# qdrant/qdrant

Measured on AMD Instinct MI355X. Metric: QPS @ recall@10, brute-force, d=768 10M vecs, f32 cosine top-10, higher is better.
Workload: dtype f32 (int8 prefilter + exact f32 re-score)

## Files before the change

### qdrant_amd/csrc/api_core.hip

```cpp
#include "api_internal.hpp"

namespace qmx {

static thread_local std::string g_last_error;
const std::string &last_error_text() { return g_last_error; }

void set_error(const char *fmt, ...) {
    char buf[1024];
    va_list ap;
    va_start(ap, fmt);
    vsnprintf(buf, sizeof(buf), fmt, ap);
    va_end(ap);
    g_last_error = buf;
}

int32_t hip_status(hipError_t e, const char *what, const char *file, int line) {
    set_error("HIP error %d (%s) at %s:%d: %s", (int)e, hipGetErrorString(e), file, line, what);
    (void)hipGetLastError();
    switch (e) {
        case hipErrorOutOfMemory: return QMX_ERR_OUT_OF_MEMORY;
        case hipErrorNoDevice:
        case hipErrorInvalidDevice:
        case hipErrorNoBinaryForGpu:
        case hipErrorInsufficientDriver: return QMX_ERR_NO_DEVICE;
        case hipErrorNotReady: return QMX_ERR_NOT_READY;
        case hipErrorInvalidValue: return QMX_ERR_BAD_ARG;
        default: return QMX_ERR_OTHER;
    }
}

static const char *const g_option_names[OPT_COUNT] = {"no_mfma_scan", "no_mfma16", "no_prescan", "prescan_shift", "hnsw_log_cap", "no_split_scan", "split_min_queries", "no_split256", "no_pq_pair", "no_pq_prefilter", "pq_prefilter_min_queries", "hnsw_pq_per_cu", "tq_rotate_block", "no_topk_small", "verify_max_per_query", "hnsw_pq_direct_walk", "hnsw_pq_table_build", "hnsw_no_pq_prefilter", "hnsw_no_lds_visited", "pq_lut_no_lds", "hnsw_per_cu", "hnsw_reference_heap_order", "tq_wide_min_queries", "tq_wide_high_digit", "sq_wide_min_queries", "i8_resident", "i8_dense_epilogue", "i8_sample_stride", "prescan_beside_scan", "group_matrix_bytes", "debug"};
struct OptionTable {
    std::atomic<int64_t> v[OPT_COUNT];
    int64_t initial[OPT_COUNT];
    OptionTable() {
        for (int i = 0; i < OPT_COUNT; ++i) {
            char env[64] = "QMX_";
            size_t k = 4;
            for (const char *c = g_option_names[i]; *c && k + 1 < sizeof(env); ++c) env[k++] = (char)toupper((unsigned char)*c);
            env[k] = 0;
            const char *e = getenv(env);
            int64_t val = 0;
            if (e) { val = (*e >= '0' && *e <= '9') ? atoll(e) : 1; }
            if (i == OPT_PRESCAN_SHIFT && !e) val = 10;
            if (i == OPT_SPLIT_MIN_QUERIES && !e) val = 1;
            if (i == OPT_PQ_PREFILTER_MIN_QUERIES && !e) val = 4;
            if (i == OPT_TQ_WIDE_MIN_QUERIES && !e) val = 33;
            if (i == OPT_SQ_WIDE_MIN_QUERIES && !e) val = 33;
            if (i == OPT_I8_RESIDENT && !e) val = 1;
            if (i == OPT_I8_DENSE_EPILOGUE && !e) val = 1;
            if (i == OPT_I8_SAMPLE_STRIDE && !e) val = 16;
            if (i == OPT_PRESCAN_BESIDE_SCAN && !e) val = 1;
            initial[i] = val;
            v[i].store(val, std::memory_order_relaxed);
        }
    }
};
static OptionTable g_options;
int64_t option(Option o) { return g_options.v[o].load(std::memory_order_relaxed); }

static thread_local const void *g_last_kernel = nullptr;
const void *last_noted_kernel() { return g_last_kernel; }
void note_kernel(const void *host_function) { g_last_kernel = host_function; }

void clear_stale_error() {
    hipError_t e = hipGetLastError();
    if (e != hipSuccess) {
        const bool debug = option(OPT_DEBUG) != 0;
        if (debug) fprintf(stderr, "[qmx] dropped stale HIP error %d (%s) before a kernel launch\n", (int)e, hipGetErrorString(e));
    }
}

bool is_device_ptr(const void *p) {
    if (!p) return false;
// ... 91 lines not shown
```

### qdrant_amd/csrc/api_internal.hpp

```cpp
#pragma once
#include <stdarg.h>
#include <stdio.h>
#include <stdlib.h>
#include <string.h>

#include <ctype.h>
#include <cxxabi.h>

#include <algorithm>
#include <atomic>
#include <mutex>
#include <string>
#include <thread>
#include <new>
#include <vector>

#include "kernels.hpp"
#include "dev_mem.hpp"
#include "tq_rotate.hpp"

namespace qmx {
const std::string &last_error_text();
const void *last_noted_kernel();
bool is_device_ptr(const void *p);
// ... 123 lines not shown
    uint32_t timing_launches = 0;
    DevBuf partial, out, counts, ids, scores, misc, enc, bounds, gthr;
    DevBuf mv_qfirst, mv_offsets, mv_deleted;
    DevBuf cq_multi;
    DevBuf cq_sims, cq_scores, cq_desc, cq_coefs;
    uint32_t n_cq_coefs = 0;
    DevBuf cand, cand_cnt, cand_ids;
    DevBuf mmr_ids, mmr_rel;
    DevBuf grp_state, grp_pages, grp_scores, grp_queries, grp_partial, grp_out;
    DevBuf mmr_spill;
    DevBuf sp_bq, sp_f32, sp_cand, sp_cnt, sp_ver, sp_vscores, sp_sample, sp_wl, xcnt, tq_rot;
    DevBuf sh_lists, sh_out;
    std::vector<uint32_t> sh_bases_host;
    hipEvent_t sh_done = nullptr;
    hipEvent_t sh_merged = nullptr;
    DevBuf pq_table;
    DevBuf sp_probe, sp_pscores;
    DevBuf sp_plan, sp_fq;
    qmx_counters last_counters{};
    bool last_split = false, last_pq = false;
    uint32_t last_fqt = 64;
    uint64_t last_row_bytes = 0, last_n_cand = 0;
    uint64_t sp_sample_n = 0, sp_sample_of = 0;
    DevBuf filter;
    uint64_t n_filter_bits = 0;
    bool has_filter = false;
    DevBuf filter_of, filter_of_packed;
    uint32_t n_filters = 0;
    uint64_t filter_stride = 0;
    bool has_filters = false;
    DevBuf hnsw_lutx;
    DevBuf hnsw_pq8;
    DevBuf hnsw_next;
    DevBuf hnsw_refc;
    DevBuf hnsw_vis, hnsw_log, hnsw_scored;
    uint32_t hnsw_slots = 0;
    uint64_t hnsw_vis_words = 0;
    int *d_err = nullptr;
    uint32_t partial_grid_cap = 0;
    bool timing = false;
    const void *last_kernel = nullptr;
    SparseQuery *sparse = nullptr;

    qmx_query() = default;
    qmx_query(const qmx_query &) = delete;
    qmx_query &operator=(const qmx_query &) = delete;
// ... 284 lines not shown
```

### qdrant_amd/csrc/api_search.hip

```cpp
#include "api_internal.hpp"

extern "C" {

struct SearchCall {
    qmx_query *q;
    uint32_t top;
    const uint32_t *d_ids;
    uint64_t n_cand;
    qmx_scored_point *d_out;
    uint32_t *d_counts;
    const volatile uint8_t *is_stopped;
    qmx_counters *counters;
    bool timed;
    uint32_t launches;
};

static ScanArgs tile_args(const qmx_query *q, uint32_t top, uint64_t n_cand, uint32_t tile0, uint32_t nq_tile) {
    ScanArgs a;
    fill_args(q, tile0, nq_tile, a);
    a.n_cand = n_cand;
    a.top = top;
    return a;
}
static ScanArgs tile_args(const SearchCall &c, uint32_t tile0, uint32_t nq_tile) { return tile_args(c.q, c.top, c.n_cand, tile0, nq_tile); }
// ... 69 lines not shown
    hipError_t e = hipStreamSynchronize(q->stream);
    fprintf(stderr, "[qmx] split stage %-28s %s\n", what, e == hipSuccess ? "ok" : hipGetErrorString(e));
    fflush(stderr);
    QMX_HIP(e);
    return QMX_OK;
}

static int32_t verify_pool(qmx_query *q, unsigned char *plan, VerifyPool *vp) {
    const uint32_t cap = (uint32_t)std::min<uint64_t>(std::max<uint64_t>((uint64_t)q->nq * SPLIT_VCAP, 262144), 1u << 26);
    QMX_TRY(q->sp_ver.reserve(((size_t)cap * 2 + (size_t)q->nq * 2) * 4));
    QMX_TRY(q->sp_vscores.reserve((size_t)cap * 4));
    uint32_t *b = (uint32_t *)q->sp_ver.p;
    const int64_t mx = option(OPT_VERIFY_MAX_PER_QUERY);
    *vp = VerifyPool{b, b + cap, b + (size_t)2 * cap, b + (size_t)2 * cap + q->nq, (uint32_t *)(plan + SplitPlanLayout::pool_used), cap,
                     mx > 0 ? (uint32_t)std::min<int64_t>(mx, cap) : cap};
    return QMX_OK;
}

__global__ void sample_ids_kernel(uint32_t *ids, uint32_t n, uint64_t step) {
    const uint32_t i = blockIdx.x * blockDim.x + threadIdx.x;
    if (i < n) ids[i] = (uint32_t)((uint64_t)i * step);
}

static int32_t prefilter_begin(qmx_query *q, const SplitPlanLayout &pl, uint64_t n_cand, int shift, VerifyPool *vp, uint64_t *S_out) {
    QMX_TRY(q->sp_plan.reserve(pl.bytes));
    QMX_TRY(verify_pool(q, (unsigned char *)q->sp_plan.p, vp));
    const int sshift = (int)std::min<int64_t>(std::max<int64_t>(option(OPT_PRESCAN_SHIFT) + shift, 1), 20);
    const uint64_t S = std::min<uint64_t>(n_cand, std::max<uint64_t>(n_cand >> sshift, 8192));
    if (q->sp_sample_n != S || q->sp_sample_of != n_cand) {
        QMX_TRY(q->sp_sample.reserve((size_t)S * 4));
        ::qmx::clear_stale_error();
        hipLaunchKernelGGL(sample_ids_kernel, dim3((uint32_t)((S + 255) / 256)), dim3(256), 0, q->stream, (uint32_t *)q->sp_sample.p, (uint32_t)S, n_cand / S);
        QMX_HIP(hipGetLastError());
        q->sp_sample_n = S;
        q->sp_sample_of = n_cand;
    }
    QMX_HIP(hipMemsetAsync(q->sp_plan.p, 0, pl.zero_bytes, q->stream));
    *S_out = S;
    return QMX_OK;
}

static int32_t bound_enqueue(const SearchCall &c, uint32_t tile0, uint32_t nq_tile, const uint32_t *d_ids, uint64_t n, uint32_t ktop, const DeletedView &del,
                             uint32_t *launches, bool sample) {
    qmx_query *q = c.q;
    QMX_TRY(q->scores.reserve((size_t)nq_tile * n * sizeof(float)));
    QMX_TRY(score_matrix_enqueue(q, tile0, nq_tile, d_ids, n, (float *)q->scores.p, n, launches, sample));
    return launch_custom_topk(q->stream, (const float *)q->scores.p, n, d_ids, del, nq_tile, ktop, c.d_out + (size_t)tile0 * c.top, c.d_counts + tile0,
                              (uint64_t *)q->gthr.p + tile0, sample);
}

static int32_t verify_and_sort(const SearchCall &c, const VerifyPool &vp, uint32_t nq) {
    qmx_query *q = c.q;
    const void *scan_kernel = q->last_kernel;
    PairSel sel{vp.qsel, 0, nullptr, vp.used};
    QMX_TRY(score_pairs_device(q, sel, vp.ids, vp.cap, (float *)q->sp_vscores.p, false));
    q->last_kernel = scan_kernel;
    QMX_TRY(split_stage(q, "verify gather"));
    QMX_TRY(launch_sort_scored(q->stream, (const float *)q->sp_vscores.p, vp.ids, vp.cnt, 0, nq, c.top, c.d_out, c.d_counts, vp.off));
// ... 182 lines not shown
        else QMX_TIMED_SCAN(c, launch_scan_tq4w(q->stream, a, q->sp_bq.p, f.wide_thr, f.wide_qinfo, tq_high ? f.band : nullptr, s->num_cus, q->sp_wl.p, &grid));
        int *tile_ovf = (int *)(plan + pl.tile_ovf) + n_tiles;
        QMX_TRY(launch_regroup_lists(q->stream, a.del, (const unsigned char *)q->sp_wl.p + (sq ? sqw_wlists_counts_bytes(s->num_cus) : tq4w_wlists_counts_bytes(s->num_cus)),
                                     (const uint32_t *)q->sp_wl.p, sq ? sqw_wcap() : tq4w_wcap(), grid * 8, (uint64_t *)q->sp_cand.p, (uint32_t *)q->sp_cnt.p,
                                     SPLIT_CAND_CAP, tile_ovf));
        QMX_TRY(launch_split_select(q->stream, (const uint64_t *)q->sp_cand.p, (const uint32_t *)q->sp_cnt.p, SPLIT_CAND_CAP, f.band, nq_tile, c.top, vp, tile0, tile_ovf,
                                    (uint32_t *)(plan + pl.ovf_q) + tile0, (SplitStats *)plan, tq_high ? f.wide_high : nullptr, tq_high));
        c.launches += 6;
    }
    QMX_TRY(verify_and_sort(c, vp, q->nq));
    QMX_TRY(overflow_passes(c, pl, q->nq, TQW_FQT, sq ? overflow_scan_sq : overflow_scan_tq, &c.launches));
    q->last_split = true;
    q->last_pq = false;
    q->last_fqt = TQW_FQT;
    close_counters(c, (uint64_t)q->nq * c.n_cand,
                   (uint64_t)n_tiles * c.n_cand * s->row_bytes + (uint64_t)((q->nq + MAX_QT_MFMA - 1) / MAX_QT_MFMA) * S * s->row_bytes, c.launches, q->nq);
    return QMX_OK;
}

struct SplitTiles {
    SplitPlanLayout pl;
    VerifyPool vp{};
    uint64_t S = 0;
    std::vector<std::pair<uint32_t, uint32_t>> tiles;
    SplitTiles(uint32_t nq, uint32_t fqt) : pl(nq, fqt) {}
};

static inline float split_rel_band(bool half, uint32_t dim) {
    const float acc = (float)dim * 1.1920929e-7f;
    return (half ? 9.765625e-4f + 9.5367432e-7f : 1.9073486e-6f) + acc;
}

static int32_t split_begin(const SearchCall &c, const SearchPlan &plan, SplitTiles &sp) {
    qmx_query *q = c.q;
    const qmx_segment *s = q->seg;
    QMX_TRY(q->sp_bq.reserve(split_query_bytes(s->dim)));
    QMX_TRY(q->sp_f32.reserve(SplitF32::floats * sizeof(float)));
    QMX_TRY(q->sp_cand.reserve((size_t)plan.split_qt * SPLIT_CAND_CAP * sizeof(uint64_t)));
    QMX_TRY(q->sp_cnt.reserve((size_t)SPLIT_QT_MAX * 4));
    if (s->d_rows_split) QMX_TRY(q->sp_wl.reserve(split_wlists_bytes(s->num_cus)));
    QMX_TRY(q->sp_fq.reserve((size_t)sp.pl.list_cap * q->q_stride));
    if (s->split_i8) {
        QMX_TRY(q->sp_probe.reserve((size_t)q->nq * (split_i8_probe() + 1) * 4));
        QMX_TRY(q->sp_pscores.reserve((size_t)q->nq * split_i8_probe() * 4));
    }
    return prefilter_begin(q, sp.pl, c.n_cand, s->d_rows_split ? 1 : -2, &sp.vp, &sp.S);
}

static int32_t f16_split_scan(SearchCall &c, SplitTiles &sp, const ScanArgs &a, uint32_t tile0, uint32_t nq_tile, int *tile_ovf) {
    qmx_query *q = c.q;
    const qmx_segment *s = q->seg;
    unsigned char *plan = (unsigned char *)q->sp_plan.p;
    const SplitF32 f(q->sp_f32.p);
    const float row_scale = split_row_scale(s->row_maxabs);
    const int half = s->split_half ? 1 : 0;
    const uint32_t tqt = nq_tile > SPLIT_QT ? SPLIT_QT_MAX : SPLIT_QT;
    QMX_TRY(launch_split_pack_queries(q->stream, (const float *)q->enc.p + (size_t)tile0 * s->dim, nq_tile, s->dim, f.qmax, f.qnorm, q->sp_bq.p, half, tqt));
    QMX_TRY(launch_split_thresholds(q->stream, (const uint64_t *)q->gthr.p + tile0, f.qnorm, f.qmax, nq_tile, split_rel_band(half, s->dim), s->row_norm_max, row_scale,
                                    f.scales, f.thr, f.band, tqt, (uint32_t *)q->sp_cnt.p, SPLIT_QT_MAX));
    QMX_TRY(split_stage(q, "pack + thresholds"));
    for (uint32_t phase = s->d_rows_split ? 1 : 0; phase <= (s->d_rows_split ? 2u : 0u); ++phase) {
        QMX_TIMED_SCAN(c, launch_scan_f32_split(q->stream, a, q->sp_bq.p, row_scale, f.scales, f.thr, (uint64_t *)q->sp_cand.p, (uint32_t *)q->sp_cnt.p, SPLIT_CAND_CAP,
                                                s->num_cus, s->d_rows_split, half, q->sp_wl.p, phase, tqt));
        if (s->d_rows_split)
            QMX_TRY(launch_split_regroup(q->stream, a, q->sp_wl.p, s->num_cus, (uint64_t *)q->sp_cand.p, (uint32_t *)q->sp_cnt.p, SPLIT_CAND_CAP, tile_ovf, phase, tqt));
        if (phase == 1)
            QMX_TRY(launch_split_refine(q->stream, (const uint64_t *)q->sp_cand.p, (const uint32_t *)q->sp_cnt.p, SPLIT_CAND_CAP, f.band, nq_tile, c.top, f.scales, f.thr));
    }
    QMX_TRY(split_stage(q, "split kernel"));
    QMX_TRY(launch_split_select(q->stream, (const uint64_t *)q->sp_cand.p, (const uint32_t *)q->sp_cnt.p, SPLIT_CAND_CAP, f.band, nq_tile, c.top, sp.vp, tile0, tile_ovf,
                                (uint32_t *)(plan + sp.pl.ovf_q) + tile0, (SplitStats *)plan));
    c.launches += 8;
    return QMX_OK;
}

static int32_t i8_copy_scan(SearchCall &c, SplitTiles &sp, const ScanArgs &a, uint32_t tile0, uint32_t nq_tile, int *tile_ovf) {
    qmx_query *q = c.q;
    const qmx_segment *s = q->seg;
    unsigned char *plan = (unsigned char *)q->sp_plan.p;
    const SplitF32 f(q->sp_f32.p);
    QMX_TRY(launch_split_i8_pack(q->stream, (const float *)q->enc.p + (size_t)tile0 * s->dim, nq_tile, s->dim, s->d_i8_scale, (const uint64_t *)q->gthr.p + tile0,
                                 s->d_i8_stats, s->row_norm_max, q->sp_bq.p, f.i8_qscale, f.band, f.thr, f.i8_texact, (uint32_t *)q->sp_cnt.p, SPLIT_QT_MAX));
    QMX_TRY(split_stage(q, "int8 pack"));
    const uint32_t np = split_i8_probe();
    uint32_t *probe_ids = (uint32_t *)q->sp_probe.p, *probe_cnt = probe_ids + (size_t)q->nq * np;
    const int64_t sstride_opt = option(OPT_I8_SAMPLE_STRIDE);
    const uint32_t sstride = sstride_opt >= 2 && sstride_opt <= 255 ? (uint32_t)sstride_opt : 16;
    for (uint32_t ph = 1; ph <= 2; ++ph) {
        const uint32_t phase = ph | (sstride << 8);
        QMX_TIMED_SCAN(c, launch_scan_i8copy(q->stream, a, q->sp_bq.p, f.i8_qscale, f.thr, s->num_cus, s->d_rows_split, q->sp_wl.p, phase));
        QMX_TRY(launch_split_regroup(q->stream, a, q->sp_wl.p, s->num_cus, (uint64_t *)q->sp_cand.p, (uint32_t *)q->sp_cnt.p, SPLIT_CAND_CAP, tile_ovf, phase, SPLIT_QT));
        QMX_TRY(launch_split_i8_probe(q->stream, (const uint64_t *)q->sp_cand.p, (const uint32_t *)q->sp_cnt.p, SPLIT_CAND_CAP, f.band, nq_tile, c.top, tile_ovf,
                                      probe_ids + (size_t)tile0 * np, probe_cnt + tile0));
        const void *scan_kernel = q->last_kernel;
        PairSel psel{nullptr, np, probe_cnt};
        QMX_TRY(score_pairs_device(q, psel, probe_ids, (uint64_t)(tile0 + nq_tile) * np, (float *)q->sp_pscores.p, false));
        q->last_kernel = scan_kernel;
        QMX_TRY(launch_split_i8_bound(q->stream, (const float *)q->sp_pscores.p + (size_t)tile0 * np, probe_cnt + tile0, nq_tile, c.top, f.band, f.i8_qscale, f.thr,
                                      f.i8_texact));
    }
    QMX_TRY(split_stage(q, "int8 scan"));
    QMX_TRY(launch_split_select(q->stream, (const uint64_t *)q->sp_cand.p, (const uint32_t *)q->sp_cnt.p, SPLIT_CAND_CAP, f.band, nq_tile, c.top, sp.vp, tile0, tile_ovf,
                                (uint32_t *)(plan + sp.pl.ovf_q) + tile0, (SplitStats *)plan, f.i8_texact));
    c.launches += 13;
    return QMX_OK;
}

static int32_t split_tile(SearchCall &c, const SearchPlan &plan, SplitTiles &sp, uint32_t tile0, uint32_t nq_tile) {
    qmx_query *q = c.q;
    QMX_CHECK_CANCELLED(c.is_stopped);
    const ScanArgs a = tile_args(c, tile0, nq_tile);
    QMX_TRY(bound_enqueue(c, tile0, nq_tile, (const uint32_t *)q->sp_sample.p, sp.S, c.top, a.del, nullptr, true));
    QMX_TRY(split_stage(q, "prescan"));
    int *tile_ovf = (int *)((unsigned char *)q->sp_plan.p + sp.pl.tile_ovf) + sp.tiles.size();
    if (plan.route == ROUTE_I8_COPY) QMX_TRY(i8_copy_scan(c, sp, a, tile0, nq_tile, tile_ovf));
    else QMX_TRY(f16_split_scan(c, sp, a, tile0, nq_tile, tile_ovf));
    QMX_TRY(split_stage(q, "select"));
    sp.tiles.push_back({tile0, nq_tile});
    return QMX_OK;
}

static int32_t split_finish(const SearchCall &c, const SearchPlan &plan, const SplitTiles &sp) {
    qmx_query *q = c.q;
    const uint32_t first = sp.tiles.front().first, last = sp.tiles.back().first + sp.tiles.back().second;
    QMX_REQUIRE(first == 0, QMX_ERR_OTHER, "split tiles must start at query 0");
    QMX_TRY(verify_and_sort(c, sp.vp, last));
    QMX_TRY(overflow_passes(c, sp.pl, last, plan.split_fqt, overflow_scan_f32, nullptr));
    q->last_split = true;
    q->last_pq = false;
    q->last_fqt = plan.split_fqt;
    return QMX_OK;
}

static int32_t exact_tile(SearchCall &c, const SearchPlan &plan, uint32_t tile0, uint32_t nq_tile) {
    qmx_query *q = c.q;
// ... 39 lines not shown
    const SearchPlan plan = search_plan(q, top, d_ids, c.n_cand);
    q->last_counters = qmx_counters{};
    q->last_split = false;
    if (plan.route == ROUTE_TQ_L1) return tq_l1_search(c, plan);
    if (plan.route == ROUTE_PQ_PREFILTER) return pq_prefilter_search(c);
    if (plan.route == ROUTE_TQ_WIDE || plan.route == ROUTE_SQ_WIDE) return wide_exact_search(c);
    const uint32_t TQ = plan.tile_q;
    QMX_TRY(q->partial.reserve((size_t)s->num_cus * 8 * std::min<uint32_t>(TQ, MAX_QT_TOPK) * std::min<uint32_t>(top, MAX_TOP_FAST) * sizeof(uint64_t)));
    if (plan.n_pass > 1) QMX_TRY(q->bounds.reserve((size_t)TQ * sizeof(uint64_t)));
    QMX_TRY(q->gthr.reserve((size_t)std::max<uint32_t>(q->nq_padded, SPLIT_QT_MAX) * sizeof(uint64_t)));
    SplitTiles sp(q->nq, plan.split_fqt);
    if (plan.split()) QMX_TRY(split_begin(c, plan, sp));
    for (uint32_t tile0 = 0; tile0 < q->nq; tile0 += TQ) {
        const uint32_t nq_tile = std::min<uint32_t>(TQ, q->nq - tile0);
        if (plan.tile_splits(nq_tile)) QMX_TRY(split_tile(c, plan, sp, tile0, nq_tile));
        else QMX_TRY(exact_tile(c, plan, tile0, nq_tile));
    }
    if (!sp.tiles.empty()) QMX_TRY(split_finish(c, plan, sp));
    uint32_t split_q = 0;
    uint64_t bytes = 0;
    for (auto &t : sp.tiles) {
        split_q += t.second;
        bytes += c.n_cand * (uint64_t)s->dim * (s->split_i8 ? 1 : s->d_rows_split && s->split_half ? 2 : 4);
        bytes += (uint64_t)((t.second + tile_qt(s, q) - 1) / tile_qt(s, q)) * q->sp_sample_n * s->row_bytes;
    }
    bytes += (uint64_t)((q->nq - split_q + TQ - 1) / TQ) * c.n_cand * s->row_bytes * plan.n_pass;
    close_counters(c, (uint64_t)q->nq * c.n_cand * plan.n_pass, bytes, counters ? counters->kernel_launches + c.launches : 0, split_q);
    return QMX_OK;
}

int32_t fold_split_counters(qmx_query *q, qmx_counters *c) {
    if (!q->last_split || !q->sp_plan.p) return QMX_OK;
    SplitStats st;
    QMX_HIP(hipMemcpy(&st, q->sp_plan.p, sizeof(st), hipMemcpyDeviceToHost));
    c->prefilter_candidates = st.candidates;
    c->verified_rows = st.verified;
    c->fallback_queries = st.fallback_queries;
    c->bytes_read += st.verified * q->last_row_bytes;
    if (st.fallback_queries) {
        const uint32_t f = st.fallback_queries;
        const uint64_t passes = q->last_pq ? f : f <= 16 ? 1 : (f + q->last_fqt - 1) / q->last_fqt;
        c->bytes_read += passes * q->last_n_cand * q->last_row_bytes;
    }
    return QMX_OK;
}

static int32_t zero_counts(qmx_query *q, uint32_t *out_counts) {
// ... 192 lines not shown
```

### qdrant_amd/csrc/common.hpp

```cpp
#pragma once
#include <hip/hip_runtime.h>
#include <hip/hip_fp16.h>
#include <stdint.h>
#include <atomic>
#include <string>

#include "../../include/qdrant_amd.h"

namespace qmx {

void set_error(const char *fmt, ...);
int32_t hip_status(hipError_t e, const char *what, const char *file, int line);
void clear_stale_error();

enum Option {
    OPT_NO_MFMA_SCAN = 0,
    OPT_NO_MFMA16,
    OPT_NO_PRESCAN,
    OPT_PRESCAN_SHIFT,
    OPT_HNSW_LOG_CAP,
    OPT_NO_SPLIT_SCAN,
    OPT_SPLIT_MIN_QUERIES,
    OPT_NO_SPLIT256,
    OPT_NO_PQ_PAIR,
    OPT_NO_PQ_PREFILTER,
    OPT_PQ_PREFILTER_MIN_QUERIES,
    OPT_HNSW_PQ_PER_CU,
    OPT_TQ_ROTATE_BLOCK,
    OPT_NO_TOPK_SMALL,
    OPT_VERIFY_MAX_PER_QUERY,
    OPT_HNSW_PQ_DIRECT_WALK,
    OPT_HNSW_PQ_TABLE_BUILD,
    OPT_HNSW_NO_PQ_PREFILTER,
    OPT_HNSW_NO_LDS_VISITED,
    OPT_PQ_LUT_NO_LDS,
    OPT_HNSW_PER_CU,
    OPT_HNSW_REFERENCE_HEAP_ORDER,
    OPT_TQ_WIDE_MIN_QUERIES,
    OPT_TQ_WIDE_HIGH_DIGIT,
    OPT_SQ_WIDE_MIN_QUERIES,
    OPT_I8_RESIDENT,
    OPT_I8_DENSE_EPILOGUE,
    OPT_I8_SAMPLE_STRIDE,
    OPT_PRESCAN_BESIDE_SCAN,
    OPT_GROUP_MATRIX_BYTES,
    OPT_DEBUG,
    OPT_COUNT
};
int64_t option(Option o);
struct DeviceOnce {
    std::atomic<uint64_t> done{0};
    int dev = 0;
    bool need() {
        if (hipGetDevice(&dev) != hipSuccess) { dev = 0; return true; }
        return dev >= 64 || !(done.load(std::memory_order_acquire) & (1ull << dev));
    }
    void mark() { if (dev < 64) done.fetch_or(1ull << dev, std::memory_order_release); }
};
void note_kernel(const void *host_function);
#define QMX_NOTE_KERNEL(fn) ::qmx::note_kernel(reinterpret_cast<const void *>(fn))

#define QMX_HIP(expr)                                                        \
    do {                                                                     \
        hipError_t e__ = (expr);                                             \
        if (e__ != hipSuccess) return ::qmx::hip_status(e__, #expr, __FILE__, __LINE__); \
    } while (0)
// ... 116 lines not shown
```

### qdrant_amd/csrc/kernels.hpp

```cpp
#pragma once
#include "common.hpp"

namespace qmx {

constexpr int MAX_QT = 16;
constexpr int SCAN_BLOCK = 512;
constexpr int MAX_TOP_FAST = 64;

struct TqEc {
    const int16_t *weights;
    const float *xm;
    float weight_scale, mm_const;
};
struct ScanArgs {
    const void *rows;
    uint64_t n_rows;
    uint64_t row_stride;
    uint32_t dim;
    uint32_t nseg;
    uint32_t rem_pieces;
    uint32_t tail_start;
    uint32_t aux_off;
    uint32_t nq;
    const void *queries;
// ... 294 lines not shown
    uint32_t *ids, *qsel, *off, *cnt, *used;
    uint32_t cap;
    uint32_t max_per_query;
};
int32_t launch_split_select(hipStream_t st, const uint64_t *d_cand, const uint32_t *d_cand_cnt, uint32_t cap, const float *d_band, uint32_t nq, uint32_t top,
                            const VerifyPool &pool, uint32_t q_base, const int *d_tile_overflow, uint32_t *d_ovf_q, SplitStats *d_stats,
                            const float *d_t_exact = nullptr, bool tighten = false);
bool split_i8_dim_ok(uint32_t dim);
size_t split_i8_copy_bytes(uint64_t n, uint32_t dim);
size_t split_i8_query_bytes(uint32_t dim);
uint32_t split_i8_probe();
int32_t launch_split_i8_colstats(hipStream_t st, const void *rows, uint64_t row_stride, uint64_t n, uint32_t dim, uint32_t *d_colmax, float *d_colsq);
float split_i8_choose_scales(const float *colmax, const float *colsq, uint64_t n, uint32_t dim, float *scale);
int32_t launch_split_i8_rowstats(hipStream_t st, const void *rows, uint64_t row_stride, uint64_t n, uint32_t dim, const float *d_scale, uint32_t *d_stats);
int32_t launch_split_i8_copy(hipStream_t st, const void *rows, uint64_t row_stride, uint64_t n, uint32_t dim, const float *d_scale, void *d_out);
int32_t launch_split_i8_pack(hipStream_t st, const float *d_q, uint32_t nq, uint32_t dim, const float *d_scale, const uint64_t *d_gthr, const uint32_t *d_row_stats,
                             float row_norm_max, void *d_bq, float *d_qscale, float *d_band, float *d_thr, float *d_t_exact, uint32_t *d_cand_cnt, uint32_t n_cnt);
int32_t launch_scan_i8copy(hipStream_t st, const ScanArgs &a, const void *d_bq, const float *d_qscale, const float *d_thr, int num_cus, const void *d_rows_i8,
                           void *d_wlists, uint32_t phase);
int32_t launch_split_i8_probe(hipStream_t st, const uint64_t *d_cand, const uint32_t *d_cand_cnt, uint32_t cap, const float *d_band, uint32_t nq, uint32_t top,
                              const int *d_tile_overflow, uint32_t *d_probe_ids, uint32_t *d_probe_cnt);
int32_t launch_split_i8_bound(hipStream_t st, const float *d_scores, uint32_t *d_probe_cnt, uint32_t nq, uint32_t top, const float *d_band, const float *d_qscale,
                              float *d_thr, float *d_t_exact);
bool tq4w_shape_ok(const ScanArgs &a);
size_t tq4w_query_bytes(uint32_t code_bytes);
size_t tq4w_wlists_counts_bytes(int num_cus);
size_t tq4w_wlists_bytes(int num_cus);
uint32_t tq4w_wcap();
int32_t launch_tq4w_stats(hipStream_t st, const float *d_sf, const float *d_l2, const void *d_rows, uint64_t row_stride, uint32_t code_bytes, uint64_t n, uint32_t *d_stats);
int32_t launch_tq4w_pack(hipStream_t st, const ScanArgs &a, const uint64_t *d_gthr, float sf_min, float sf_max, float l2_min, float l2_max, uint32_t c1, int high_only,
                         void *d_bq, int32_t *d_thr_i,
                         float *d_qinfo, float *d_band, uint32_t *d_cand_cnt, uint32_t n_cnt);
int32_t launch_scan_tq4w(hipStream_t st, const ScanArgs &a, const void *d_bq, const int32_t *d_thr_i, const float *d_qinfo, const float *d_band_high_only, int num_cus,
                         void *d_wlists, uint32_t *grid_out);
bool sqw_shape_ok(const ScanArgs &a);
size_t sqw_query_bytes(uint32_t dim);
size_t sqw_wlists_counts_bytes(int num_cus);
size_t sqw_wlists_bytes(int num_cus);
uint32_t sqw_wcap();
int32_t launch_sqw_stats(hipStream_t st, const float *d_off, uint64_t n, float multiplier, int32_t *d_bi, uint32_t *d_stats);
int32_t launch_sqw_pack(hipStream_t st, const ScanArgs &a, const uint64_t *d_gthr, float off_absmax, void *d_bq, int32_t *d_thr_i, float *d_qinfo, float *d_band,
                        uint32_t *d_cand_cnt, uint32_t n_cnt);
int32_t launch_scan_sqw(hipStream_t st, const ScanArgs &a, const void *d_bq, const int32_t *d_thr_i, const int32_t *d_bi, const float *d_qinfo, int num_cus,
                        void *d_wlists, uint32_t *grid_out);
int32_t launch_split_plan(hipStream_t st, const uint32_t *d_ovf_q, uint32_t nq, const uint64_t *d_gthr, uint32_t *d_list, uint64_t *d_gthr_packed, uint32_t list_cap,
                          uint32_t *d_count, int *d_run16, int *d_run64, uint32_t n_run64, SplitStats *d_stats, const void *d_queries, uint32_t q_stride,
// ... 256 lines not shown
```

### qdrant_amd/csrc/scan_split.hip

```cpp
#include <type_traits>

#include "scan_common.hpp"

namespace qmx {

typedef _Float16 half8 __attribute__((ext_vector_type(8)));
typedef _Float16 half4 __attribute__((ext_vector_type(4)));
typedef float f32x4s __attribute__((ext_vector_type(4)));

constexpr int SP_BM = 256;
constexpr int SP_QT = 128;
constexpr int SP_QT_MAX = 256;
constexpr int SP_THREADS = 768;
constexpr int SP_CONSUMERS = 8;
constexpr int SP_A_UNITS = SP_BM * 2 * 4;
constexpr int SP_B_UNITS = SP_QT * 2 * 4;
constexpr int SP_BRING = 4;
constexpr int SP_LDS = (2 * SP_A_UNITS + SP_BRING * SP_B_UNITS) * 16;

__device__ __forceinline__ uint32_t sp_unit(uint32_t t, uint32_t hl, uint32_t kq, uint32_t m) { return ((t * 2 + hl) * 4 + kq) * 16 + (m ^ (2 * kq)); }

__device__ __forceinline__ void sp_split4(const f32x4s v, float scale, half4 &h, half4 &l) {
#pragma unroll
    for (int i = 0; i < 4; ++i) {
// ... 1116 lines not shown
            float c = __builtin_rintf(x);
            c = c > 127.0f ? 127.0f : (c < -127.0f ? -127.0f : c);
            if (!(c == c)) c = 0.0f;
            const float f = x - c;
            sabs += __builtin_fabsf(c);
            sf2 = __builtin_fmaf(f, f, sf2);
            w[e / 4] |= ((uint32_t)(int)c & 0xFFu) << (8 * (e % 4));
        }
        bq[(uint64_t)k128 * SP_B_UNITS + sp_unit(qi >> 4, hl, kq, qi & 15u)] = make_uint4(w[0], w[1], w[2], w[3]);
    }
    sabs = sp_block_sum(sabs, sh_red);
    sf2 = sp_block_sum(sf2, sh_red);
    if (threadIdx.x != 0) return;
    if (!live) {
        qscale[qi] = 0.0f;
        band[qi] = 0.0f;
        thr[qi] = __builtin_inff();
        t_exact[qi] = -__builtin_inff();
        return;
    }
    const float c1 = (float)row_stats[0], c2 = __builtin_sqrtf((float)row_stats[1]);
    const float cf = __builtin_fminf(0.5f * c1, c2 * __builtin_sqrtf(sf2));
    const float b = t * (cf + 0.5f * sabs + 0.25f * (float)dim) * 1.001f + 2.0f * (float)dim * 1.1920929e-7f * row_norm_max * __builtin_sqrtf(ss);
    const uint64_t k = gthr[qi];
    const bool ok = bad == 0.0f && k != 0 && b < 3.0e38f;
    qscale[qi] = t;
    band[qi] = ok ? b : __builtin_inff();
    t_exact[qi] = ok ? key_score(k) : -__builtin_inff();
    thr[qi] = ok ? (key_score(k) - b) / t : __builtin_inff();
}

constexpr int SP8_BRING = 3;
constexpr int SP8_LDS = (SP3_ARING * SP3_A_UNITS + SP8_BRING * SP_B_UNITS) * 16;
__global__ __launch_bounds__(SP3_THREADS, 1) void scan_i8copy_kernel(const ScanArgs a, const SplitArgs s) {
    extern __shared__ __attribute__((aligned(16))) unsigned char smem_raw[];
    uint4 *lds = reinterpret_cast<uint4 *>(smem_raw);
    const int tid = threadIdx.x, lane = tid & 63;
    const int w = __builtin_amdgcn_readfirstlane(tid >> 6);
    const uint64_t all_tiles = (a.n_cand + SP3_BM - 1) / SP3_BM;
    const uint64_t n_tiles = split_phase_tiles(all_tiles, s.phase);
    const uint32_t nch = s.nchunks;
    const uint64_t my_tiles = blockIdx.x < n_tiles ? (n_tiles - blockIdx.x + gridDim.x - 1) / gridDim.x : 0;
    const uint32_t phase = s.phase & 0xFFu, pstride = split_phase_stride(s.phase);
    auto tile_of = [&](uint64_t j) -> uint64_t { return phase == 0 ? j : phase == 1 ? j * pstride : j + j / (pstride - 1) + 1; };
    if (my_tiles == 0) {
        if (lane == 0) s.wcnt[blockIdx.x * (SP3_THREADS / 64) + (uint32_t)w] = 0;
        return;
    }
    const uint32_t wm = (uint32_t)w & 3u, wn = (uint32_t)w >> 2;
    const uint32_t kq_r = (uint32_t)lane >> 4, m_r = (uint32_t)lane & 15u;
// ... 410 lines not shown
            }
        }
    }
    __syncthreads();
    if (threadIdx.x == 0) probe_cnt[q] = sh_n < SP_I8_PROBE ? sh_n : SP_I8_PROBE;
}
__global__ __launch_bounds__(64) void sp_i8_bound_kernel(const float *scores, uint32_t *probe_cnt, uint32_t top, const float *band, const float *qscale,
                                                         float *thr, float *t_exact) {
    const uint32_t q = blockIdx.x;
    const int lane = threadIdx.x;
    const uint32_t n = probe_cnt[q];
    const float sc = (uint32_t)lane < n ? scores[(uint64_t)q * SP_I8_PROBE + lane] : -__builtin_inff();
    uint32_t rank = 0;
    for (int j = 0; j < 64; ++j) {
        const float o = __shfl(sc, j, 64);
        rank += (o > sc || (o == sc && j < lane)) ? 1u : 0u;
    }
    if (lane == 0) probe_cnt[q] = 0;
    if (n < top || !(band[q] < 3.0e38f)) return;
    if ((uint32_t)lane < n && rank == top - 1 && sc == sc) {
        if (sc > t_exact[q]) t_exact[q] = sc;
        const float t = (sc - band[q]) / qscale[q];
        if (t > thr[q]) thr[q] = t;
    }
}

bool split_scan_ok(const ScanArgs &a) {
    return a.dim % 128 == 0 && a.dim >= 128 && a.rem_pieces == 0 && a.tail_start == a.dim && a.row_stride % 16 == 0 && a.ids == nullptr && a.top <= 64 &&
           !option(OPT_NO_SPLIT_SCAN);
}
size_t split_wlists_counts_bytes(int num_cus) { return ((size_t)num_cus * (SP3_THREADS / 64) * 4 + 255) / 256 * 256; }
size_t split_wlists_bytes(int num_cus) { return split_wlists_counts_bytes(num_cus) + (size_t)num_cus * (SP3_THREADS / 64) * SP_WCAP * 16; }
size_t split_query_bytes(uint32_t dim) { return (size_t)(dim / 32) * SP4_B_UNITS * 16; }

int32_t launch_split_row_stats(hipStream_t st, const void *rows, uint64_t row_stride, uint64_t n, uint32_t dim, uint32_t *d_stats) {
    if (n == 0) return QMX_OK;
    ::qmx::clear_stale_error();
    hipLaunchKernelGGL(sp_row_stats_kernel, dim3(2048), dim3(256), 0, st, (const unsigned char *)rows, row_stride, n, dim, d_stats);
    QMX_HIP(hipGetLastError());
    return QMX_OK;
}
float split_row_scale(float row_maxabs) {
    if (!(row_maxabs > 0.0f) || !(row_maxabs < 3.0e38f)) return 1.0f;
    int e;
    (void)frexpf(row_maxabs, &e);
    int s = 14 - e;
// ... 251 lines not shown
    const uint64_t n_tiles = split_phase_tiles((a.n_cand + SP3_BM - 1) / SP3_BM, phase);
    if (n_tiles == 0) return QMX_OK;
    const uint32_t grid = (uint32_t)std::max<uint64_t>(1, std::min<uint64_t>(n_tiles, (uint64_t)num_cus));
    ::qmx::clear_stale_error();
    QMX_NOTE_KERNEL(kfn);
    hipLaunchKernelGGL(kfn, dim3(grid), dim3(SP3_THREADS), lds_bytes, st, a, s);
    QMX_HIP(hipGetLastError());
    return QMX_OK;
}
int32_t launch_split_i8_probe(hipStream_t st, const uint64_t *d_cand, const uint32_t *d_cand_cnt, uint32_t cap, const float *d_band, uint32_t nq, uint32_t top,
                              const int *d_tile_overflow, uint32_t *d_probe_ids, uint32_t *d_probe_cnt) {
    ::qmx::clear_stale_error();
    hipLaunchKernelGGL(sp_i8_probe_kernel, dim3(nq), dim3(SEL_BLOCK), 0, st, d_cand, d_cand_cnt, cap, d_band, d_tile_overflow, top, d_probe_ids, d_probe_cnt);
    QMX_HIP(hipGetLastError());
    return QMX_OK;
}
int32_t launch_split_i8_bound(hipStream_t st, const float *d_scores, uint32_t *d_probe_cnt, uint32_t nq, uint32_t top, const float *d_band, const float *d_qscale,
                              float *d_thr, float *d_t_exact) {
    ::qmx::clear_stale_error();
    hipLaunchKernelGGL(sp_i8_bound_kernel, dim3(nq), dim3(64), 0, st, d_scores, d_probe_cnt, top, d_band, d_qscale, d_thr, d_t_exact);
    QMX_HIP(hipGetLastError());
    return QMX_OK;
}

}
```

Before: 100,000.

## Seed int8 split-scan threshold from an int8 MFMA sample scan instead of f32 prescan

Adds an int8 sample prescan that is on by default. It scores 16-row tiles of the resident int8 copy with MFMA and takes a top-k over the sample. The picks are re-scored exactly in f32, and the k-th exact score seeds the pruning threshold and band. This replaces the f32 bound_enqueue prescan, which read full f32 rows for the sample. It adds several small launches and relies on the int8 band to keep the threshold valid.

```diff
diff --git a/qdrant_amd/csrc/api_core.hip b/qdrant_amd/csrc/api_core.hip
--- a/qdrant_amd/csrc/api_core.hip
+++ b/qdrant_amd/csrc/api_core.hip
@@ -29,7 +29,7 @@
     }
 }
 
-static const char *const g_option_names[OPT_COUNT] = {"no_mfma_scan", "no_mfma16", "no_prescan", "prescan_shift", "hnsw_log_cap", "no_split_scan", "split_min_queries", "no_split256", "no_pq_pair", "no_pq_prefilter", "pq_prefilter_min_queries", "hnsw_pq_per_cu", "tq_rotate_block", "no_topk_small", "verify_max_per_query", "hnsw_pq_direct_walk", "hnsw_pq_table_build", "hnsw_no_pq_prefilter", "hnsw_no_lds_visited", "pq_lut_no_lds", "hnsw_per_cu", "hnsw_reference_heap_order", "tq_wide_min_queries", "tq_wide_high_digit", "sq_wide_min_queries", "i8_resident", "i8_dense_epilogue", "i8_sample_stride", "prescan_beside_scan", "group_matrix_bytes", "debug"};
+static const char *const g_option_names[OPT_COUNT] = {"no_mfma_scan", "no_mfma16", "no_prescan", "prescan_shift", "hnsw_log_cap", "no_split_scan", "split_min_queries", "no_split256", "no_pq_pair", "no_pq_prefilter", "pq_prefilter_min_queries", "hnsw_pq_per_cu", "tq_rotate_block", "no_topk_small", "verify_max_per_query", "hnsw_pq_direct_walk", "hnsw_pq_table_build", "hnsw_no_pq_prefilter", "hnsw_no_lds_visited", "pq_lut_no_lds", "hnsw_per_cu", "hnsw_reference_heap_order", "tq_wide_min_queries", "tq_wide_high_digit", "sq_wide_min_queries", "i8_resident", "i8_dense_epilogue", "i8_sample_stride", "i8_sample_scan", "i8_sample_rows", "prescan_beside_scan", "group_matrix_bytes", "debug"};
 struct OptionTable {
     std::atomic<int64_t> v[OPT_COUNT];
     int64_t initial[OPT_COUNT];
@@ -50,6 +50,7 @@
             if (i == OPT_I8_RESIDENT && !e) val = 1;
             if (i == OPT_I8_DENSE_EPILOGUE && !e) val = 1;
             if (i == OPT_I8_SAMPLE_STRIDE && !e) val = 16;
+            if (i == OPT_I8_SAMPLE_SCAN && !e) val = 1;
             if (i == OPT_PRESCAN_BESIDE_SCAN && !e) val = 1;
             initial[i] = val;
             v[i].store(val, std::memory_order_relaxed);
diff --git a/qdrant_amd/csrc/api_internal.hpp b/qdrant_amd/csrc/api_internal.hpp
--- a/qdrant_amd/csrc/api_internal.hpp
+++ b/qdrant_amd/csrc/api_internal.hpp
@@ -169,6 +169,7 @@
     uint32_t last_fqt = 64;
     uint64_t last_row_bytes = 0, last_n_cand = 0;
     uint64_t sp_sample_n = 0, sp_sample_of = 0;
+    bool sp_sample_tiles = false;
     DevBuf filter;
     uint64_t n_filter_bits = 0;
     bool has_filter = false;
diff --git a/qdrant_amd/csrc/api_search.hip b/qdrant_amd/csrc/api_search.hip
--- a/qdrant_amd/csrc/api_search.hip
+++ b/qdrant_amd/csrc/api_search.hip
@@ -115,18 +115,34 @@
     if (i < n) ids[i] = (uint32_t)((uint64_t)i * step);
 }
 
-static int32_t prefilter_begin(qmx_query *q, const SplitPlanLayout &pl, uint64_t n_cand, int shift, VerifyPool *vp, uint64_t *S_out) {
+__global__ void sample_tile_ids_kernel(uint32_t *ids, uint32_t n, uint64_t step) {
+    const uint32_t i = blockIdx.x * blockDim.x + threadIdx.x;
+    if (i < n) ids[i] = (uint32_t)((uint64_t)(i >> 4) * step * 16u + (i & 15u));
+}
+
+static int32_t prefilter_begin(qmx_query *q, const SplitPlanLayout &pl, uint64_t n_cand, int shift, VerifyPool *vp, uint64_t *S_out, bool tiles = false) {
     QMX_TRY(q->sp_plan.reserve(pl.bytes));
     QMX_TRY(verify_pool(q, (unsigned char *)q->sp_plan.p, vp));
     const int sshift = (int)std::min<int64_t>(std::max<int64_t>(option(OPT_PRESCAN_SHIFT) + shift, 1), 20);
-    const uint64_t S = std::min<uint64_t>(n_cand, std::max<uint64_t>(n_cand >> sshift, 8192));
-    if (q->sp_sample_n != S || q->sp_sample_of != n_cand) {
+    uint64_t S = std::min<uint64_t>(n_cand, std::max<uint64_t>(n_cand >> sshift, 8192));
+    if (tiles) {
+        const int64_t rows_opt = option(OPT_I8_SAMPLE_ROWS);
+        if (rows_opt > 0) S = std::min<uint64_t>(n_cand, std::max<int64_t>(rows_opt, 16));
+        S &= ~(uint64_t)15;
+        QMX_REQUIRE(S >= 16, QMX_ERR_OTHER, "a sample of row tiles needs a block of 16 rows");
+    }
+    if (q->sp_sample_n != S || q->sp_sample_of != n_cand || q->sp_sample_tiles != tiles) {
         QMX_TRY(q->sp_sample.reserve((size_t)S * 4));
         ::qmx::clear_stale_error();
-        hipLaunchKernelGGL(sample_ids_kernel, dim3((uint32_t)((S + 255) / 256)), dim3(256), 0, q->stream, (uint32_t *)q->sp_sample.p, (uint32_t)S, n_cand / S);
+        if (tiles)
+            hipLaunchKernelGGL(sample_tile_ids_kernel, dim3((uint32_t)((S + 255) / 256)), dim3(256), 0, q->stream, (uint32_t *)q->sp_sample.p, (uint32_t)S,
+                               (n_cand / 16) / (S / 16));
+        else
+            hipLaunchKernelGGL(sample_ids_kernel, dim3((uint32_t)((S + 255) / 256)), dim3(256), 0, q->stream, (uint32_t *)q->sp_sample.p, (uint32_t)S, n_cand / S);
         QMX_HIP(hipGetLastError());
         q->sp_sample_n = S;
         q->sp_sample_of = n_cand;
+        q->sp_sample_tiles = tiles;
     }
     QMX_HIP(hipMemsetAsync(q->sp_plan.p, 0, pl.zero_bytes, q->stream));
     *S_out = S;
@@ -355,6 +371,7 @@
     SplitPlanLayout pl;
     VerifyPool vp{};
     uint64_t S = 0;
+    bool i8_sample = false;
     std::vector<std::pair<uint32_t, uint32_t>> tiles;
     SplitTiles(uint32_t nq, uint32_t fqt) : pl(nq, fqt) {}
 };
@@ -377,7 +394,8 @@
         QMX_TRY(q->sp_probe.reserve((size_t)q->nq * (split_i8_probe() + 1) * 4));
         QMX_TRY(q->sp_pscores.reserve((size_t)q->nq * split_i8_probe() * 4));
     }
-    return prefilter_begin(q, sp.pl, c.n_cand, s->d_rows_split ? 1 : -2, &sp.vp, &sp.S);
+    sp.i8_sample = s->split_i8 && option(OPT_I8_SAMPLE_SCAN) > 0;
+    return prefilter_begin(q, sp.pl, c.n_cand, s->d_rows_split ? 1 : -2, &sp.vp, &sp.S, sp.i8_sample);
 }
 
 static int32_t f16_split_scan(SearchCall &c, SplitTiles &sp, const ScanArgs &a, uint32_t tile0, uint32_t nq_tile, int *tile_ovf) {
@@ -412,11 +430,29 @@
     const qmx_segment *s = q->seg;
     unsigned char *plan = (unsigned char *)q->sp_plan.p;
     const SplitF32 f(q->sp_f32.p);
-    QMX_TRY(launch_split_i8_pack(q->stream, (const float *)q->enc.p + (size_t)tile0 * s->dim, nq_tile, s->dim, s->d_i8_scale, (const uint64_t *)q->gthr.p + tile0,
-                                 s->d_i8_stats, s->row_norm_max, q->sp_bq.p, f.i8_qscale, f.band, f.thr, f.i8_texact, (uint32_t *)q->sp_cnt.p, SPLIT_QT_MAX));
+    QMX_TRY(launch_split_i8_pack(q->stream, (const float *)q->enc.p + (size_t)tile0 * s->dim, nq_tile, s->dim, s->d_i8_scale,
+                                 sp.i8_sample ? nullptr : (const uint64_t *)q->gthr.p + tile0, s->d_i8_stats, s->row_norm_max, q->sp_bq.p, f.i8_qscale, f.band, f.thr,
+                                 f.i8_texact, (uint32_t *)q->sp_cnt.p, SPLIT_QT_MAX));
     QMX_TRY(split_stage(q, "int8 pack"));
     const uint32_t np = split_i8_probe();
     uint32_t *probe_ids = (uint32_t *)q->sp_probe.p, *probe_cnt = probe_ids + (size_t)q->nq * np;
+    if (sp.i8_sample) {
+        QMX_TRY(q->scores.reserve((size_t)nq_tile * sp.S * sizeof(float)));
+        QMX_TRY(launch_scan_i8copy_sample(q->stream, s->d_rows_split, q->sp_bq.p, s->dim, (const uint32_t *)q->sp_sample.p, (uint32_t)(sp.S / 16), nq_tile, f.i8_qscale,
+                                          (float *)q->scores.p));
+        QMX_TRY(launch_custom_topk(q->stream, (const float *)q->scores.p, sp.S, (const uint32_t *)q->sp_sample.p, a.del, nq_tile, c.top, c.d_out + (size_t)tile0 * c.top,
+                                   c.d_counts + tile0, nullptr, true));
+        QMX_TRY(launch_split_i8_picks(q->stream, c.d_out + (size_t)tile0 * c.top, c.d_counts + tile0, nq_tile, c.top, f.band, probe_ids + (size_t)tile0 * np,
+                                      probe_cnt + tile0));
+        const void *scan_kernel = q->last_kernel;
+        PairSel psel{nullptr, np, probe_cnt};
+        QMX_TRY(score_pairs_device(q, psel, probe_ids, (uint64_t)(tile0 + nq_tile) * np, (float *)q->sp_pscores.p, false));
+        q->last_kernel = scan_kernel;
+        QMX_TRY(launch_split_i8_sample_bound(q->stream, (const float *)q->sp_pscores.p + (size_t)tile0 * np, probe_ids + (size_t)tile0 * np, probe_cnt + tile0, nq_tile,
+                                             c.top, f.band, f.i8_qscale, f.thr, f.i8_texact, (uint64_t *)q->gthr.p + tile0));
+        QMX_TRY(split_stage(q, "int8 sample scan"));
+        c.launches += 3;
+    }
     const int64_t sstride_opt = option(OPT_I8_SAMPLE_STRIDE);
     const uint32_t sstride = sstride_opt >= 2 && sstride_opt <= 255 ? (uint32_t)sstride_opt : 16;
     for (uint32_t ph = 1; ph <= 2; ++ph) {
@@ -443,7 +479,7 @@
     qmx_query *q = c.q;
     QMX_CHECK_CANCELLED(c.is_stopped);
     const ScanArgs a = tile_args(c, tile0, nq_tile);
-    QMX_TRY(bound_enqueue(c, tile0, nq_tile, (const uint32_t *)q->sp_sample.p, sp.S, c.top, a.del, nullptr, true));
+    if (!sp.i8_sample) QMX_TRY(bound_enqueue(c, tile0, nq_tile, (const uint32_t *)q->sp_sample.p, sp.S, c.top, a.del, nullptr, true));
     QMX_TRY(split_stage(q, "prescan"));
     int *tile_ovf = (int *)((unsigned char *)q->sp_plan.p + sp.pl.tile_ovf) + sp.tiles.size();
     if (plan.route == ROUTE_I8_COPY) QMX_TRY(i8_copy_scan(c, sp, a, tile0, nq_tile, tile_ovf));
@@ -529,7 +565,11 @@
     for (auto &t : sp.tiles) {
         split_q += t.second;
         bytes += c.n_cand * (uint64_t)s->dim * (s->split_i8 ? 1 : s->d_rows_split && s->split_half ? 2 : 4);
-        bytes += (uint64_t)((t.second + tile_qt(s, q) - 1) / tile_qt(s, q)) * q->sp_sample_n * s->row_bytes;
+        if (sp.i8_sample) {
+            const uint32_t group = split_i8_sample_queries(s->dim, t.second);
+            bytes += (uint64_t)((t.second + group - 1) / group) * q->sp_sample_n * s->dim + (uint64_t)t.second * std::min<uint32_t>(top, MAX_TOP_FAST) * s->row_bytes;
+        } else
+            bytes += (uint64_t)((t.second + tile_qt(s, q) - 1) / tile_qt(s, q)) * q->sp_sample_n * s->row_bytes;
     }
     bytes += (uint64_t)((q->nq - split_q + TQ - 1) / TQ) * c.n_cand * s->row_bytes * plan.n_pass;
     close_counters(c, (uint64_t)q->nq * c.n_cand * plan.n_pass, bytes, counters ? counters->kernel_launches + c.launches : 0, split_q);
diff --git a/qdrant_amd/csrc/common.hpp b/qdrant_amd/csrc/common.hpp
--- a/qdrant_amd/csrc/common.hpp
+++ b/qdrant_amd/csrc/common.hpp
@@ -42,6 +42,8 @@
     OPT_I8_RESIDENT,
     OPT_I8_DENSE_EPILOGUE,
     OPT_I8_SAMPLE_STRIDE,
+    OPT_I8_SAMPLE_SCAN,
+    OPT_I8_SAMPLE_ROWS,
     OPT_PRESCAN_BESIDE_SCAN,
     OPT_GROUP_MATRIX_BYTES,
     OPT_DEBUG,
diff --git a/qdrant_amd/csrc/kernels.hpp b/qdrant_amd/csrc/kernels.hpp
--- a/qdrant_amd/csrc/kernels.hpp
+++ b/qdrant_amd/csrc/kernels.hpp
@@ -340,6 +340,13 @@
                               const int *d_tile_overflow, uint32_t *d_probe_ids, uint32_t *d_probe_cnt);
 int32_t launch_split_i8_bound(hipStream_t st, const float *d_scores, uint32_t *d_probe_cnt, uint32_t nq, uint32_t top, const float *d_band, const float *d_qscale,
                               float *d_thr, float *d_t_exact);
+uint32_t split_i8_sample_queries(uint32_t dim, uint32_t nq);
+int32_t launch_scan_i8copy_sample(hipStream_t st, const void *d_rows_i8, const void *d_bq, uint32_t dim, const uint32_t *d_sample, uint32_t n_tiles, uint32_t nq,
+                                  const float *d_qscale, float *d_scores);
+int32_t launch_split_i8_picks(hipStream_t st, const qmx_scored_point *d_lists, const uint32_t *d_counts, uint32_t nq, uint32_t top, const float *d_band,
+                              uint32_t *d_probe_ids, uint32_t *d_probe_cnt);
+int32_t launch_split_i8_sample_bound(hipStream_t st, const float *d_scores, const uint32_t *d_probe_ids, uint32_t *d_probe_cnt, uint32_t nq, uint32_t top,
+                                     float *d_band, const float *d_qscale, float *d_thr, float *d_t_exact, uint64_t *d_gthr);
 bool tq4w_shape_ok(const ScanArgs &a);
 size_t tq4w_query_bytes(uint32_t code_bytes);
 size_t tq4w_wlists_counts_bytes(int num_cus);
diff --git a/qdrant_amd/csrc/scan_split.hip b/qdrant_amd/csrc/scan_split.hip
--- a/qdrant_amd/csrc/scan_split.hip
+++ b/qdrant_amd/csrc/scan_split.hip
@@ -1162,10 +1162,11 @@
     const float c1 = (float)row_stats[0], c2 = __builtin_sqrtf((float)row_stats[1]);
     const float cf = __builtin_fminf(0.5f * c1, c2 * __builtin_sqrtf(sf2));
     const float b = t * (cf + 0.5f * sabs + 0.25f * (float)dim) * 1.001f + 2.0f * (float)dim * 1.1920929e-7f * row_norm_max * __builtin_sqrtf(ss);
-    const uint64_t k = gthr[qi];
-    const bool ok = bad == 0.0f && k != 0 && b < 3.0e38f;
+    const uint64_t k = gthr ? gthr[qi] : 0;
+    const bool finite = bad == 0.0f && b < 3.0e38f;
+    const bool ok = finite && k != 0;
     qscale[qi] = t;
-    band[qi] = ok ? b : __builtin_inff();
+    band[qi] = (gthr ? ok : finite) ? b : __builtin_inff();
     t_exact[qi] = ok ? key_score(k) : -__builtin_inff();
     thr[qi] = ok ? (key_score(k) - b) / t : __builtin_inff();
 }
@@ -1622,6 +1623,125 @@
         if (sc > t_exact[q]) t_exact[q] = sc;
         const float t = (sc - band[q]) / qscale[q];
         if (t > thr[q]) thr[q] = t;
+    }
+}
+
+template <int NQ>
+__global__ __launch_bounds__(256) void scan_i8copy_sample_kernel(const uint4 *rows_i8, const uint4 *bq, uint32_t nch, const uint32_t *sample_ids, uint32_t n_tiles,
+                                                                 uint32_t nq, const float *qscale, float *scores) {
+    constexpr int NT = NQ / 16, MT = 2, NL = 2 * MT;
+    static_assert(NQ == 16 || NQ == 32 || NQ == 64, "whole query tiles, a divisor of the 128-query tile");
+    extern __shared__ __attribute__((aligned(16))) unsigned char smem_raw[];
+    uint4 *lds = reinterpret_cast<uint4 *>(smem_raw);
+    const int tid = threadIdx.x, lane = tid & 63;
+    const uint32_t w = (uint32_t)__builtin_amdgcn_readfirstlane(tid >> 6);
+    const uint32_t q0 = blockIdx.y * NQ;
+    for (uint32_t u = (uint32_t)tid; u < nch * (NT * 128u); u += 256) {
+        const uint32_t kc = u / (NT * 128u), r = u % (NT * 128u);
+        lds[u] = bq[(uint64_t)kc * SP_B_UNITS + (q0 / 16u) * 128u + r];
+    }
+    __syncthreads();
+    const uint32_t t0 = (blockIdx.x * 4u + w) * MT;
+    if (t0 >= n_tiles) return;
+    const bool two = t0 + 1 < n_tiles;
+    const unsigned char *base[MT];
+#pragma unroll
+    for (int mt = 0; mt < MT; ++mt) {
+        const uint32_t rt = (uint32_t)__builtin_amdgcn_readfirstlane((int)(sample_ids[(uint64_t)(two ? t0 + (uint32_t)mt : t0) * 16u] >> 4));
+        base[mt] = reinterpret_cast<const unsigned char *>(rows_i8) + ((uint64_t)(rt >> 4) * nch) * (SP3_A_UNITS * 16u) + (rt & 15u) * 2048u;
+    }
+    asm volatile("s_waitcnt vmcnt(0) lgkmcnt(0)" ::: "memory");
+    const uint32_t kq_r = (uint32_t)lane >> 4, m_r = (uint32_t)lane & 15u;
+    const uint32_t lane_unit = kq_r * 16u + (m_r ^ (2u * kq_r));
+    const uint4 *const b_rd = lds + lane_unit;
+    const uint32_t lane_off = lane_unit * 16u;
+    auto load_stage = [&](uint32_t kc, i32x4s (&rc)[NL]) __attribute__((always_inline)) {
+        const uint64_t off = (uint64_t)(kc < nch ? kc : nch - 1) * (SP3_A_UNITS * 16u);
+        sp_gload16<0>(rc[0], base[0] + off, lane_off);
+        sp_gload16<1024>(rc[1], base[0] + off, lane_off);
+        sp_gload16<0>(rc[2], base[1] + off, lane_off);
+        sp_gload16<1024>(rc[3], base[1] + off, lane_off);
+    };
+    i32x4s acc[MT][NT];
+#pragma unroll
+    for (int mt = 0; mt < MT; ++mt)
+#pragma unroll
+        for (int nt = 0; nt < NT; ++nt) acc[mt][nt] = (i32x4s){0, 0, 0, 0};
+    auto landed = [](i32x4s (&rc)[NL]) __attribute__((always_inline)) { asm volatile("" : "+v"(rc[0]), "+v"(rc[1]), "+v"(rc[2]), "+v"(rc[3]) : : "memory"); };
+    auto one_stage = [&](uint32_t kc, const i32x4s (&cur)[NL]) __attribute__((always_inline)) {
+#pragma unroll
+        for (int hl = 0; hl < 2; ++hl) {
+            const uint4 *bb = b_rd + (size_t)kc * (NT * 128u) + hl * 64;
+#pragma unroll
+            for (int nt = 0; nt < NT; ++nt) {
+                const i32x4s bv = *reinterpret_cast<const i32x4s *>(bb + nt * 128);
+#pragma unroll
+                for (int mt = 0; mt < MT; ++mt) acc[mt][nt] = __builtin_amdgcn_mfma_i32_16x16x64_i8(cur[mt * 2 + hl], bv, acc[mt][nt], 0, 0, 0);
+            }
+        }
+        __builtin_amdgcn_sched_barrier(0);
+    };
+    i32x4s ra[NL], rb[NL];
+    for (uint32_t kc = 0; kc < nch; kc += 2) {
+        load_stage(kc, ra);
+        load_stage(kc + 1, rb);
+        asm volatile("s_waitcnt vmcnt(%0)" : : "n"(NL) : "memory");
+        landed(ra);
+        one_stage(kc, ra);
+        asm volatile("s_waitcnt vmcnt(0)" ::: "memory");
+        landed(rb);
+        if (kc + 1 < nch) one_stage(kc + 1, rb);
+    }
+    const uint64_t S = (uint64_t)n_tiles * 16u;
+#pragma unroll
+    for (int nt = 0; nt < NT; ++nt) {
+        const uint32_t q = q0 + (uint32_t)nt * 16u + m_r;
+        if (q >= nq) continue;
+        const float qs = qscale[q];
+#pragma unroll
+        for (int mt = 0; mt < MT; ++mt) {
+            if (mt == 1 && !two) continue;
+            float4 v;
+            v.x = (float)acc[mt][nt][0] * qs;
+            v.y = (float)acc[mt][nt][1] * qs;
+            v.z = (float)acc[mt][nt][2] * qs;
+            v.w = (float)acc[mt][nt][3] * qs;
+            *reinterpret_cast<float4 *>(scores + (uint64_t)q * S + (uint64_t)(t0 + (uint32_t)mt) * 16u + 4u * kq_r) = v;
+        }
+    }
+}
+__global__ __launch_bounds__(64) void sp_i8_picks_kernel(const qmx_scored_point *lists, const uint32_t *counts, uint32_t top, const float *band, uint32_t *probe_ids,
+                                                         uint32_t *probe_cnt) {
+    const uint32_t q = blockIdx.x, lane = threadIdx.x;
+    uint32_t n = counts[q] < top ? counts[q] : top;
+    n = n < SP_I8_PROBE ? n : SP_I8_PROBE;
+    if (!(band[q] < 3.0e38f)) n = 0;
+    if (lane < n) probe_ids[(uint64_t)q * SP_I8_PROBE + lane] = lists[(uint64_t)q * top + lane].idx;
+    if (lane == 0) probe_cnt[q] = n;
+}
+__global__ __launch_bounds__(64) void sp_i8_sample_bound_kernel(const float *scores, const uint32_t *probe_ids, uint32_t *probe_cnt, uint32_t top, float *band,
+                                                                const float *qscale, float *thr, float *t_exact, uint64_t *gthr) {
+    const uint32_t q = blockIdx.x;
+    const int lane = threadIdx.x;
+    const uint32_t n = probe_cnt[q];
+    const float sc = (uint32_t)lane < n ? scores[(uint64_t)q * SP_I8_PROBE + lane] : 0.0f;
+    const uint64_t key = (uint32_t)lane < n && sc == sc ? make_key(sc, probe_ids[(uint64_t)q * SP_I8_PROBE + lane]) : 0ull;
+    uint32_t rank = 0;
+    for (int j = 0; j < 64; ++j) rank += (uint64_t)__shfl((unsigned long long)key, j, 64) > key ? 1u : 0u;
+    if (lane == 0) probe_cnt[q] = 0;
+    const bool finite = band[q] < 3.0e38f;
+    const bool mine = finite && n >= top && key != 0 && rank == top - 1;
+    if (!__ballot(mine)) {
+        if (lane == 0) {
+            band[q] = __builtin_inff();
+            gthr[q] = 0;
+        }
+        return;
+    }
+    if (mine) {
+        t_exact[q] = sc;
+        thr[q] = (sc - band[q]) / qscale[q];
+        gthr[q] = key;
     }
 }
 
@@ -1919,5 +2039,45 @@
     QMX_HIP(hipGetLastError());
     return QMX_OK;
 }
-
-}
+uint32_t split_i8_sample_queries(uint32_t dim, uint32_t nq) {
+    const uint32_t nch = dim / 128;
+    if (nch > SP8R_MAX_NCH) return 16;
+    const size_t free_lds = (size_t)160 * 1024 - sp8r_lds_bytes(nch);
+    uint32_t pick = 16;
+    for (uint32_t c = 32; c <= 64; c *= 2)
+        if ((size_t)nch * (c / 16) * 2048 <= free_lds && c / 2 < nq) pick = c;
+    return pick;
+}
+int32_t launch_scan_i8copy_sample(hipStream_t st, const void *d_rows_i8, const void *d_bq, uint32_t dim, const uint32_t *d_sample, uint32_t n_tiles, uint32_t nq,
+                                  const float *d_qscale, float *d_scores) {
+    QMX_REQUIRE(d_rows_i8 && split_i8_dim_ok(dim) && nq >= 1 && nq <= (uint32_t)SP_QT && n_tiles >= 1, QMX_ERR_BAD_ARG, "int8 sample scan of %u queries", nq);
+    const uint32_t nch = dim / 128, NQ = split_i8_sample_queries(dim, nq);
+    const size_t lds_bytes = (size_t)nch * (NQ / 16) * 2048;
+    QMX_REQUIRE(lds_bytes <= 65536, QMX_ERR_OTHER, "int8 sample scan: %zu B of query images", lds_bytes);
+    const dim3 grid((n_tiles + 7) / 8, (nq + NQ - 1) / NQ);
+    ::qmx::clear_stale_error();
+    if (NQ == 64)
+        hipLaunchKernelGGL(scan_i8copy_sample_kernel<64>, grid, dim3(256), lds_bytes, st, (const uint4 *)d_rows_i8, (const uint4 *)d_bq, nch, d_sample, n_tiles, nq, d_qscale, d_scores);
+    else if (NQ == 32)
+        hipLaunchKernelGGL(scan_i8copy_sample_kernel<32>, grid, dim3(256), lds_bytes, st, (const uint4 *)d_rows_i8, (const uint4 *)d_bq, nch, d_sample, n_tiles, nq, d_qscale, d_scores);
+    else
+        hipLaunchKernelGGL(scan_i8copy_sample_kernel<16>, grid, dim3(256), lds_bytes, st, (const uint4 *)d_rows_i8, (const uint4 *)d_bq, nch, d_sample, n_tiles, nq, d_qscale, d_scores);
+    QMX_HIP(hipGetLastError());
+    return QMX_OK;
+}
+int32_t launch_split_i8_picks(hipStream_t st, const qmx_scored_point *d_lists, const uint32_t *d_counts, uint32_t nq, uint32_t top, const float *d_band,
+                              uint32_t *d_probe_ids, uint32_t *d_probe_cnt) {
+    ::qmx::clear_stale_error();
+    hipLaunchKernelGGL(sp_i8_picks_kernel, dim3(nq), dim3(64), 0, st, d_lists, d_counts, top, d_band, d_probe_ids, d_probe_cnt);
+    QMX_HIP(hipGetLastError());
+    return QMX_OK;
+}
+int32_t launch_split_i8_sample_bound(hipStream_t st, const float *d_scores, const uint32_t *d_probe_ids, uint32_t *d_probe_cnt, uint32_t nq, uint32_t top,
+                                     float *d_band, const float *d_qscale, float *d_thr, float *d_t_exact, uint64_t *d_gthr) {
+    ::qmx::clear_stale_error();
+    hipLaunchKernelGGL(sp_i8_sample_bound_kernel, dim3(nq), dim3(64), 0, st, d_scores, d_probe_ids, d_probe_cnt, top, d_band, d_qscale, d_thr, d_t_exact, d_gthr);
+    QMX_HIP(hipGetLastError());
+    return QMX_OK;
+}
+
+}
```

Result: faster. 102,200 (median of 6 runs) (+2.2%).
